# batra-mlp-lab/visdial

Hardware: NVIDIA H100
Metric: QA-rounds/sec mn-att-ques-im-hist+disc train step (higher is better)
Workload: dtype f16 operands + f16 saved state for the option LSTM, tf32 operands elsewhere; fp32 accumulate, fp32 cell state / gradients / optimiser

## Files before the change

visdial_b200/csrc/lstm16.cu:

```cuda
#include <cuda.h>
#include <cuda_fp16.h>
#include <map>
#include <mutex>
#include "../../include/visdial_b200.h"
#include "kernels.cuh"
#include "tc_ptx.cuh"

namespace vd {
namespace tc {

constexpr int BM16 = 128;
constexpr int BK16 = 64;
constexpr int UK16 = 16;
constexpr int BN16 = 128;
constexpr int EW16 = 8;
constexpr int STAGE16 = 32768;

__device__ __forceinline__ float tanh16(float x) { float y; asm("tanh.approx.f32 %0, %1;" : "=f"(y) : "f"(x)); return y; }
__device__ __forceinline__ float sig16(float x) { return fmaf(0.5f, tanh16(0.5f * x), 0.5f); }

__device__ __forceinline__ uint32_t pack2(float a, float b) {
  uint32_t r;
  asm("{\n .reg .f16 lo, hi;\n cvt.rn.satfinite.f16.f32 lo, %1;\n cvt.rn.satfinite.f16.f32 hi, %2;\n mov.b32 %0, {lo, hi};\n}"
      : "=r"(r) : "f"(a), "f"(b));
  return r;
}
__device__ __forceinline__ uint4 pack8(const float* v) {
  return make_uint4(pack2(v[0], v[1]), pack2(v[2], v[3]), pack2(v[4], v[5]), pack2(v[6], v[7]));
}
__device__ __forceinline__ void unpack8(const uint4 u, float* v) {
  const __half2* h = reinterpret_cast<const __half2*>(&u);
#pragma unroll
  for (int i = 0; i < 4; ++i) { const float2 f = __half22float2(h[i]); v[2 * i] = f.x; v[2 * i + 1] = f.y; }
}

constexpr int T16_BYTES = 1024, T32_BYTES = 2048;
__device__ __forceinline__ uint8_t* t16_at(uint8_t* base, int row, int unit) {
  return base + row * 64 + (((unit >> 3) ^ ((row >> 1) & 3)) << 4) + (unit & 7) * 2;
}
__device__ __forceinline__ uint8_t* t32_at(uint8_t* base, int row, int unit) {
  return base + row * 128 + (((unit >> 2) ^ (row & 7)) << 4) + (unit & 3) * 4;
}
__device__ __forceinline__ const void* shfl_vptr(const void* p, int src_lane) {
  unsigned long long v = (unsigned long long)p;
  unsigned lo = __shfl_sync(0xffffffffu, (unsigned)v, src_lane), hi = __shfl_sync(0xffffffffu, (unsigned)(v >> 32), src_lane);
  return (const void*)(((unsigned long long)hi << 32) | lo);
}
__device__ __forceinline__ void cp16(void* dst, const void* src) {
  asm volatile("cp.async.cg.shared.global [%0], [%1], 16;" ::"r"(smem_u32(dst)), "l"(src) : "memory");
}
__device__ __forceinline__ void t16_load(uint8_t* base, const void* mine, int lane) {
#pragma unroll
  for (int ps = 0; ps < 2; ++ps) {
    const int row = ps * 8 + (lane >> 2), c = lane & 3;
    const uint8_t* src = (const uint8_t*)shfl_vptr(mine, row);
    uint8_t* dst = base + row * 64 + ((c ^ ((row >> 1) & 3)) << 4);
    if (src) cp16(dst, src + c * 16); else *reinterpret_cast<uint4*>(dst) = make_uint4(0, 0, 0, 0);
  }
}
__device__ __forceinline__ void t32_load(uint8_t* base, const void* mine, int lane) {
#pragma unroll
  for (int ps = 0; ps < 4; ++ps) {
    const int row = ps * 4 + (lane >> 3), c = lane & 7;
    const uint8_t* src = (const uint8_t*)shfl_vptr(mine, row);
    uint8_t* dst = base + row * 128 + ((c ^ (row & 7)) << 4);
    if (src) cp16(dst, src + c * 16); else *reinterpret_cast<float4*>(dst) = make_float4(0.f, 0.f, 0.f, 0.f);
  }
}
__device__ __forceinline__ void cp_wait_all() {
  asm volatile("cp.async.wait_all;" ::: "memory");
  __syncwarp();
}
__device__ __forceinline__ float2 ld_h2(uint8_t* p) { return __half22float2(*reinterpret_cast<const __half2*>(p)); }
__device__ __forceinline__ void st_h2(uint8_t* p, float a, float b) { *reinterpret_cast<uint32_t*>(p) = pack2(a, b); }

struct Lstm16Params {
  int R, H;
  const __half* ptable; const int32_t* tok;
  const float* bias;
  const float* c_prev;
  const int32_t* mask_ids;
  float* h32_out;
  int save_gates;
  const __half* gsave; const float* c_cur; float* dc_carry;
};
struct Lstm16Maps { CUtensorMap g16, c, h16; };

template <int MODE>
struct Cfg16 {
  static constexpr int THREADS = 128 + 32 * EW16;
  static constexpr int STG_PER_WARP = MODE == 0 ? (5 * T16_BYTES + T32_BYTES) : (4 * T16_BYTES + 3 * T32_BYTES);
  static constexpr int STG_BYTES = EW16 * STG_PER_WARP;
  static constexpr int STAGES = (232448 - 1024 - 256 - STG_BYTES) / STAGE16;
  static constexpr int TOTAL = STAGES * STAGE16 + STG_BYTES + 1024 + 256;
};

template <int MODE>
__global__ void __launch_bounds__(Cfg16<MODE>::THREADS, 1)
k_lstm16(const __grid_constant__ CUtensorMap tmA, const __grid_constant__ CUtensorMap tmB,
         const __grid_constant__ Lstm16Maps em, const Lstm16Params p) {
  using C = Cfg16<MODE>;
  constexpr int STAGES = C::STAGES;
  extern __shared__ uint8_t smem_raw[];
  uint8_t* smem = (uint8_t*)(((uintptr_t)smem_raw + 1023) & ~(uintptr_t)1023);
  uint8_t* stg_all = smem + STAGES * STAGE16;
  uint64_t* full = (uint64_t*)(stg_all + C::STG_BYTES);
  uint64_t* empty = full + STAGES;

  const int warp = threadIdx.x >> 5, lane = threadIdx.x & 31;
  const int H = p.H;
  const int num_m = (p.R + BM16 - 1) / BM16;
  const int num_n = MODE == 0 ? H / 32 : H / BN16;
  const int num_tiles = num_m * num_n;
  const int num_kb = (MODE == 0 ? H : 4 * H) / BK16;

  if (threadIdx.x == 0) {
    for (int s = 0; s < STAGES; ++s) { mbar_init(&full[s], 1); mbar_init(&empty[s], 2); }
    asm volatile("fence.mbarrier_init.release.cluster;" ::: "memory");
  }
  __syncthreads();

  if (warp < 4) {
    if (threadIdx.x == 0) {
      int s = 0; uint32_t ph = 0;
      for (int tile = blockIdx.x; tile < num_tiles; tile += gridDim.x) {
        const int m0 = (tile / num_n) * BM16;
        const int nt = tile % num_n;
        for (int kb = 0; kb < num_kb; ++kb) {
          mbar_wait(&empty[s], ph ^ 1);
          uint8_t* sa = smem + s * STAGE16;
          uint8_t* sb = sa + 16384;
          mbar_expect_tx(&full[s], STAGE16);
          tma_load_2d(sa, &tmA, &full[s], kb * BK16, m0);
          if (MODE == 0) {
#pragma unroll
            for (int g = 0; g < 4; ++g) tma_load_2d(sb + g * 4096, &tmB, &full[s], kb * BK16, g * H + nt * 32);
          } else {
            tma_load_2d(sb, &tmB, &full[s], kb * BK16, nt * BN16);
          }
          if (++s == STAGES) { s = 0; ph ^= 1; }
        }
      }
    }
  } else {
    const int cw = warp - 4, wg = cw >> 2;
    uint8_t* stg = stg_all + cw * C::STG_PER_WARP;
    const int fr = lane >> 2, fu = 2 * (lane & 3);
    int s = 0; uint32_t ph = 0;
    auto contract = [&](float (&d)[BN16 / 2]) {
#pragma unroll
      for (int i = 0; i < BN16 / 2; ++i) d[i] = 0.f;
      int prev = -1;
      for (int kb = 0; kb < num_kb; ++kb) {
        mbar_wait(&full[s], ph);
        const uint32_t sa = smem_u32(smem + s * STAGE16);
        const uint64_t adesc = make_desc(sa + wg * 64 * 128, 16, 1024), bdesc = make_desc(sa + 16384, 16, 1024);
        wgmma_fence();
#pragma unroll
        for (int k = 0; k < BK16 / UK16; ++k)
          wgmma_f16_n128(d, adesc + (uint64_t)(k * 2), bdesc + (uint64_t)(k * 2), (kb | k) ? 1u : 0u);
        wgmma_commit();
        wgmma_wait<1>();
        if (prev >= 0 && (threadIdx.x & 127) == 0) mbar_arrive(&empty[prev]);
        prev = s;
        if (++s == STAGES) { s = 0; ph ^= 1; }
      }
      wgmma_wait<0>();
      wgmma_hold(d);
      if (prev >= 0 && (threadIdx.x & 127) == 0) mbar_arrive(&empty[prev]);
    };
    if constexpr (MODE == 0) {
      uint8_t* sG = stg; uint8_t* sH = stg + 4 * T16_BYTES; uint8_t* sC = sH + T16_BYTES;
      for (int tile = blockIdx.x; tile < num_tiles; tile += gridDim.x) {
        const int m0 = (tile / num_n) * BM16;
        const int nt = tile % num_n;
        const int r0 = m0 + wg * 64 + (cw & 3) * 16;
        const int j0 = nt * 32;
        const int64_t row = (int64_t)r0 + (lane & 15);
        const bool row_ok = row < p.R;
        const float keep = (row_ok && p.mask_ids && p.mask_ids[row] == 0) ? 0.f : 1.f;
        const int32_t tk = row_ok ? __ldg(p.tok + row) : 0;
        const __half* prow = tk != 0 ? p.ptable + (int64_t)tk * 4 * H + j0 : nullptr;
        const float* cprow = (row_ok && p.c_prev) ? p.c_prev + row * H + j0 : nullptr;
        if (lane == 0) bulk_wait_read0();
        __syncwarp();
#pragma unroll
        for (int g = 0; g < 4; ++g) t16_load(sG + g * T16_BYTES, prow ? prow + g * H : nullptr, lane);
        t32_load(sC, cprow, lane);
        float d[BN16 / 2];
        contract(d);
        cp_wait_all();
#pragma unroll
        for (int hh = 0; hh < 2; ++hh) {
          const int r = fr + 8 * hh;
          const float kp = __shfl_sync(0xffffffffu, keep, r);
          const int64_t grow = (int64_t)r0 + r;
#pragma unroll
          for (int jj = 0; jj < 4; ++jj) {
            const int u = 8 * jj + fu;
            float a[4][2], cp[2], hn[2];
#pragma unroll
            for (int g = 0; g < 4; ++g) {
              const float2 x = ld_h2(t16_at(sG + g * T16_BYTES, r, u));
              const float2 b = __ldg(reinterpret_cast<const float2*>(p.bias + g * H + j0 + u));
              a[g][0] = d[4 * (jj + 4 * g) + 2 * hh] + (x.x + b.x);
              a[g][1] = d[4 * (jj + 4 * g) + 2 * hh + 1] + (x.y + b.y);
            }
            const float2 c2 = *reinterpret_cast<const float2*>(t32_at(sC, r, u));
            cp[0] = c2.x; cp[1] = c2.y;
#pragma unroll
            for (int e = 0; e < 2; ++e) {
              const float gi = sig16(a[0][e]), gf = sig16(a[1][e]), go = sig16(a[2][e]), gg = tanh16(a[3][e]);
              const float c_ = (gf * cp[e] + gi * gg) * kp;
              a[0][e] = gi * kp; a[1][e] = gf * kp; a[2][e] = go * kp; a[3][e] = gg * kp;
              cp[e] = c_; hn[e] = go * tanh16(c_) * kp;
            }
#pragma unroll
            for (int g = 0; g < 4; ++g) st_h2(t16_at(sG + g * T16_BYTES, r, u), a[g][0], a[g][1]);
            *reinterpret_cast<float2*>(t32_at(sC, r, u)) = make_float2(cp[0], cp[1]);
            st_h2(t16_at(sH, r, u), hn[0], hn[1]);
            if (p.h32_out && grow < p.R)
              *reinterpret_cast<float2*>(p.h32_out + grow * H + j0 + u) = make_float2(hn[0], hn[1]);
          }
        }
        fence_proxy_async_smem();
        __syncwarp();
        if (lane == 0) {
          if (p.save_gates) {
#pragma unroll
            for (int g = 0; g < 4; ++g) tma_store_2d(&em.g16, sG + g * T16_BYTES, g * H + j0, r0);
          }
          tma_store_2d(&em.c, sC, j0, r0);
          tma_store_2d(&em.h16, sH, j0, r0);
          bulk_commit();
        }
        __syncwarp();
      }
    } else {
      uint8_t* sG = stg; uint8_t* sCP = stg + 4 * T16_BYTES; uint8_t* sCC = sCP + T32_BYTES; uint8_t* sDC = sCC + T32_BYTES;
      for (int tile = blockIdx.x; tile < num_tiles; tile += gridDim.x) {
        const int m0 = (tile / num_n) * BM16;
        const int nt = tile % num_n;
        const int r0 = m0 + wg * 64 + (cw & 3) * 16;
        const int64_t row = (int64_t)r0 + (lane & 15);
        const bool row_ok = row < p.R;
        const float keep = (row_ok && p.mask_ids && p.mask_ids[row] == 0) ? 0.f : 1.f;
        const __half* grow = row_ok ? p.gsave + row * 4 * H : nullptr;
        const float* cprow = (row_ok && p.c_prev) ? p.c_prev + row * H : nullptr;
        const float* ccrow = row_ok ? p.c_cur + row * H : nullptr;
        const float* dcrow = row_ok ? p.dc_carry + row * H : nullptr;
        auto fetch = [&](int j) {
          if (lane == 0) bulk_wait_read0();
          __syncwarp();
#pragma unroll
          for (int g = 0; g < 4; ++g) t16_load(sG + g * T16_BYTES, grow ? grow + g * H + j : nullptr, lane);
          t32_load(sCP, cprow ? cprow + j : nullptr, lane);
          t32_load(sCC, ccrow ? ccrow + j : nullptr, lane);
          t32_load(sDC, dcrow ? dcrow + j : nullptr, lane);
        };
        fetch(nt * BN16);
        float d[BN16 / 2];
        contract(d);
#pragma unroll
        for (int grp = 0; grp < BN16 / 32; ++grp) {
          const int j = nt * BN16 + grp * 32;
          if (grp > 0) fetch(j);
          cp_wait_all();
#pragma unroll
          for (int hh = 0; hh < 2; ++hh) {
            const int r = fr + 8 * hh;
            const float keep_r = __shfl_sync(0xffffffffu, keep, r);
#pragma unroll
            for (int jj = 0; jj < 4; ++jj) {
              const int u = 8 * jj + fu;
              float g[4][2], cp[2], cc[2], dc[2], out[4][2], dcn[2];
#pragma unroll
              for (int gg = 0; gg < 4; ++gg) {
                const float2 x = ld_h2(t16_at(sG + gg * T16_BYTES, r, u));
                g[gg][0] = x.x; g[gg][1] = x.y;
              }
              const float2 cp2 = *reinterpret_cast<const float2*>(t32_at(sCP, r, u));
              const float2 cc2 = *reinterpret_cast<const float2*>(t32_at(sCC, r, u));
              const float2 dc2 = *reinterpret_cast<const float2*>(t32_at(sDC, r, u));
              cp[0] = cp2.x; cp[1] = cp2.y; cc[0] = cc2.x; cc[1] = cc2.y; dc[0] = dc2.x; dc[1] = dc2.y;
#pragma unroll
              for (int e = 0; e < 2; ++e) {
                const float dh = d[4 * (4 * grp + jj) + 2 * hh + e];
                const float gi = g[0][e], gf = g[1][e], go = g[2][e], gg_ = g[3][e];
                const float tcv = tanh16(cc[e]);
                const float dd = (dc[e] + dh * go * (1.f - tcv * tcv)) * keep_r;
                const float dhe = dh * keep_r;
                out[0][e] = dd * gg_ * gi * (1.f - gi);
                out[1][e] = dd * cp[e] * gf * (1.f - gf);
                out[2][e] = dhe * tcv * go * (1.f - go);
                out[3][e] = dd * gi * (1.f - gg_ * gg_);
                dcn[e] = dd * gf;
              }
#pragma unroll
              for (int gg = 0; gg < 4; ++gg) st_h2(t16_at(sG + gg * T16_BYTES, r, u), out[gg][0], out[gg][1]);
              *reinterpret_cast<float2*>(t32_at(sDC, r, u)) = make_float2(dcn[0], dcn[1]);
            }
          }
          fence_proxy_async_smem();
          __syncwarp();
          if (lane == 0) {
#pragma unroll
            for (int gg = 0; gg < 4; ++gg) tma_store_2d(&em.g16, sG + gg * T16_BYTES, gg * H + j, r0);
            tma_store_2d(&em.c, sDC, j, r0);
            bulk_commit();
          }
          __syncwarp();
        }
      }
    }
    if (lane == 0) asm volatile("cp.async.bulk.wait_group 0;" ::: "memory");
  }
}

constexpr int A16_KB = 64;
constexpr int A16_BM = 128, A16_BN = 256;
constexpr int A16_THREADS = 384;
constexpr int A16_A_BYTES = (A16_BM / 64) * A16_KB * 128;
constexpr int A16_B_BYTES = (A16_BN / 64) * A16_KB * 128;
constexpr int A16_STAGE = A16_A_BYTES + A16_B_BYTES;
constexpr int A16_STAGES = 4;
constexpr int A16_TOTAL = A16_STAGES * A16_STAGE + 1024 + 256;
constexpr int A16_CHUNKS_PER_CTA = 24;
constexpr int A16_MIN_CHUNK = 32;
struct Atb16Params {
  int M, N, tiles_n, tiles, kbt;
  int chunk, num_chunks;
  float* C; int64_t ldc; const float* inv_scale;
  int* counter;
};

template <bool VEC4>
__global__ void __launch_bounds__(A16_THREADS, 1)
k_atb16(const __grid_constant__ CUtensorMap tmA, const __grid_constant__ CUtensorMap tmB, const Atb16Params p) {
  extern __shared__ uint8_t smem_raw[];
  uint8_t* smem = (uint8_t*)(((uintptr_t)smem_raw + 1023) & ~(uintptr_t)1023);
  uint64_t* full = (uint64_t*)(smem + A16_STAGES * A16_STAGE);
  uint64_t* empty = full + A16_STAGES;
  int* tag = (int*)(empty + A16_STAGES);
  const int warp = threadIdx.x >> 5;

  if (threadIdx.x == 0) {
    for (int s = 0; s < A16_STAGES; ++s) { mbar_init(&full[s], 1); mbar_init(&empty[s], 2); }
    asm volatile("fence.mbarrier_init.release.cluster;" ::: "memory");
  }
  __syncthreads();

  if (warp < 4) {
    if (threadIdx.x == 0) {
      int s = 0; uint32_t ph = 0;
      for (;;) {
        const int c = atomicAdd(p.counter, 1);
        if (c >= p.num_chunks) break;
        const int tile = c % p.tiles, kb0 = (c / p.tiles) * p.chunk, kb1 = min(p.kbt, kb0 + p.chunk);
        const int m0 = (tile / p.tiles_n) * A16_BM, n0 = (tile % p.tiles_n) * A16_BN;
        for (int kb = kb0; kb < kb1; ++kb) {
          const int krow = kb * A16_KB;
          mbar_wait(&empty[s], ph ^ 1);
          uint8_t* sa = smem + s * A16_STAGE;
          uint8_t* sb = sa + A16_A_BYTES;
          if (kb == kb0) tag[s] = c;
          mbar_expect_tx(&full[s], A16_STAGE);
#pragma unroll
          for (int b = 0; b < A16_BM / 64; ++b) tma_load_2d(sa + b * A16_KB * 128, &tmA, &full[s], m0 + b * 64, krow);
// ... 211 lines not shown
      float* o = out + (int64_t)tok * ncols + c0;
      red_add_v4(o, acc[0] * sc, acc[1] * sc, acc[2] * sc, acc[3] * sc);
      red_add_v4(o + 4, acc[4] * sc, acc[5] * sc, acc[6] * sc, acc[7] * sc);
    };
    for (int64_t p = p0; p < p1; ++p) {
      const int tok = sorted_tok[p];
      if (tok != cur) {
        flush(cur);
#pragma unroll
        for (int e = 0; e < 8; ++e) acc[e] = 0.f;
        cur = tok;
      }
      float v[8];
      unpack8(__ldcs(reinterpret_cast<const uint4*>(X + (int64_t)perm[p] * ldx + c0)), v);
#pragma unroll
      for (int e = 0; e < 8; ++e) acc[e] += v[e];
    }
    flush(cur);
  }
}

static CUtensorMap make_tmap16(const void* base, CUtensorMapDataType dt, int esize, int64_t rows, int64_t cols, int64_t ld,
                               int box_rows, int box_cols, CUtensorMapSwizzle swz) {
  CUtensorMap tm;
  cuuint64_t dims[2] = {(cuuint64_t)cols, (cuuint64_t)rows};
  cuuint64_t strides[1] = {(cuuint64_t)ld * esize};
  cuuint32_t box[2] = {(cuuint32_t)box_cols, (cuuint32_t)box_rows};
  cuuint32_t estr[2] = {1, 1};
  CUresult r = get_encode()(&tm, dt, 2, (void*)base, dims, strides, box, estr, CU_TENSOR_MAP_INTERLEAVE_NONE, swz,
                            CU_TENSOR_MAP_L2_PROMOTION_L2_256B, CU_TENSOR_MAP_FLOAT_OOB_FILL_NONE);
  if (r != CUDA_SUCCESS) {
    char buf[256];
    snprintf(buf, sizeof(buf), "cuTensorMapEncodeTiled (lstm16) failed (%d): base %p rows %lld cols %lld ld %lld box %dx%d", (int)r, base,
             (long long)rows, (long long)cols, (long long)ld, box_rows, box_cols);
    throw CudaError(-3, buf);
  }
  return tm;
}
static CUtensorMap tmap_h(const __half* base, int64_t rows, int64_t cols, int64_t ld, int box_rows, int box_cols,
                          CUtensorMapSwizzle swz) {
  return make_tmap16(base, CU_TENSOR_MAP_DATA_TYPE_FLOAT16, 2, rows, cols, ld, box_rows, box_cols, swz);
}
static CUtensorMap tmap_f(const float* base, int64_t rows, int64_t cols, int64_t ld, int box_rows, int box_cols,
                          CUtensorMapSwizzle swz) {
  return make_tmap16(base, CU_TENSOR_MAP_DATA_TYPE_FLOAT32, 4, rows, cols, ld, box_rows, box_cols, swz);
}

template <int MODE>
static void launch16(LaunchCtx& cx, const CUtensorMap& tA, const CUtensorMap& tB, const Lstm16Maps& em, const Lstm16Params& p,
                     int num_tiles) {
  using C = Cfg16<MODE>;
  static bool attr_set = false;
  if (!attr_set) {
    VD_CUDA_CHECK(cudaFuncSetAttribute(k_lstm16<MODE>, cudaFuncAttributeMaxDynamicSharedMemorySize, C::TOTAL));
    attr_set = true;
  }
  const int pmax = cx.sms();
  int grid = num_tiles;
  if (num_tiles > pmax) { const int rounds = cdiv(num_tiles, pmax); grid = cdiv(num_tiles, rounds); }
  k_lstm16<MODE><<<grid, C::THREADS, C::TOTAL, cx.stream>>>(tA, tB, em, p);
  check_launch(cx, "k_lstm16");
}

}

bool lstm16_shape_ok(int64_t R, int H) { return H % 256 == 0 && H <= 512 && R >= 1024; }

void lstm16_step_fwd(LaunchCtx& cx, int64_t R, int H, const __half* h_prev16, const __half* Wh16, const __half* ptable16,
                     const int32_t* tok, const float* bias, const float* c_prev, const int32_t* mask_ids, __half* gates16,
                     float* c_out, __half* h16_out, float* h32_out) {
  using namespace tc;
  VD_REQUIRE(lstm16_shape_ok(R, H), VD_E_STATE, "lstm16_step_fwd: shape");
  Lstm16Params p = {};
  p.R = (int)R; p.H = H; p.ptable = ptable16; p.tok = tok; p.bias = bias; p.c_prev = c_prev; p.mask_ids = mask_ids;
  p.h32_out = h32_out; p.save_gates = gates16 != nullptr;
  CUtensorMap tA = tmap_h(h_prev16, R, H, H, BM16, BK16, CU_TENSOR_MAP_SWIZZLE_128B);
  CUtensorMap tB = tmap_h(Wh16, 4 * (int64_t)H, H, H, 32, BK16, CU_TENSOR_MAP_SWIZZLE_128B);
  Lstm16Maps em;
  em.g16 = gates16 ? tmap_h(gates16, R, 4 * (int64_t)H, 4 * (int64_t)H, 16, 32, CU_TENSOR_MAP_SWIZZLE_64B)
                   : tmap_h(h16_out, R, H, H, 16, 32, CU_TENSOR_MAP_SWIZZLE_64B);
  em.c = tmap_f(c_out, R, H, H, 16, 32, CU_TENSOR_MAP_SWIZZLE_128B);
  em.h16 = tmap_h(h16_out, R, H, H, 16, 32, CU_TENSOR_MAP_SWIZZLE_64B);
  launch16<0>(cx, tA, tB, em, p, cdiv(R, BM16) * (H / 32));
}

void lstm16_step_bwd(LaunchCtx& cx, int64_t R, int H, const __half* da_next16, const __half* Whb16, const __half* gates16,
                     const float* c_prev, const float* c_cur, float* dc_carry, const int32_t* mask_ids, __half* da16) {
  using namespace tc;
  VD_REQUIRE(lstm16_shape_ok(R, H), VD_E_STATE, "lstm16_step_bwd: shape");
  Lstm16Params p = {};
  p.R = (int)R; p.H = H; p.gsave = gates16; p.c_prev = c_prev; p.c_cur = c_cur; p.dc_carry = dc_carry; p.mask_ids = mask_ids;
  CUtensorMap tA = tmap_h(da_next16, R, 4 * (int64_t)H, 4 * (int64_t)H, BM16, BK16, CU_TENSOR_MAP_SWIZZLE_128B);
  CUtensorMap tB = tmap_h(Whb16, H, 4 * (int64_t)H, 4 * (int64_t)H, 128, BK16, CU_TENSOR_MAP_SWIZZLE_128B);
  Lstm16Maps em;
  em.g16 = tmap_h(da16, R, 4 * (int64_t)H, 4 * (int64_t)H, 16, 32, CU_TENSOR_MAP_SWIZZLE_64B);
  em.c = tmap_f(dc_carry, R, H, H, 16, 32, CU_TENSOR_MAP_SWIZZLE_128B);
  em.h16 = em.c;
  launch16<1>(cx, tA, tB, em, p, cdiv(R, BM16) * (H / BN16));
}

void lstm16_first_step(LaunchCtx& cx, int64_t R, int H, const __half* ptable16, const int32_t* tok, const float* bias,
                       const float* c_prev, const int32_t* mask_ids, __half* gates16, float* c_out, __half* h16_out, float* h32_out) {
  const int64_t n = R * (H / 8);
  tc::k_lstm16_first<<<(unsigned)((n + 255) / 256), 256, 0, cx.stream>>>(ptable16, tok, bias, c_prev, mask_ids, gates16, c_out,
                                                                          h16_out, h32_out, R, H);
  check_launch(cx, "k_lstm16_first");
}

void lstm16_bwd_last(LaunchCtx& cx, int64_t R, int H, const __half* gates16, const float* c_prev, const float* c_cur,
                     const float* dh_last, const float* scale, const int32_t* mask_ids, float* dc_carry, __half* da16) {
  const int64_t n = R * (H / 8);
  tc::k_lstm16_bwd_last<<<(unsigned)((n + 255) / 256), 256, 0, cx.stream>>>(gates16, c_prev, c_cur, dh_last, scale, mask_ids,
                                                                             dc_carry, da16, R, H);
  check_launch(cx, "k_lstm16_bwd_last");
}

void cvt_f32_to_f16(LaunchCtx& cx, __half* dst, int64_t ldd, const float* src, int64_t lds, int64_t rows, int cols) {
  VD_REQUIRE(cols % 4 == 0 && lds % 4 == 0 && ldd % 4 == 0, VD_E_STATE, "cvt_f32_to_f16: alignment");
  const int64_t n = rows * (cols / 4);
  if (n == 0) return;
  tc::k_cvt16<<<(unsigned)((n + 255) / 256), 256, 0, cx.stream>>>(dst, ldd, src, lds, rows, cols);
  check_launch(cx, "k_cvt16");
}

void pick_grad_scale(LaunchCtx& cx, const float* x, int64_t n, uint32_t* bits, float* scale2) {
  VD_REQUIRE(n % 4 == 0, VD_E_STATE, "pick_grad_scale: n % 4");
  VD_CUDA_CHECK(cudaMemsetAsync(bits, 0, sizeof(uint32_t), cx.stream));
  const int blocks = (int)std::min<int64_t>((n / 4 + 255) / 256, 4 * cx.sm_count);
  tc::k_amax<<<blocks, 256, 0, cx.stream>>>(x, n / 4, bits);
  check_launch(cx, "k_amax");
  tc::k_pick_scale<<<1, 1, 0, cx.stream>>>(bits, scale2);
  check_launch(cx, "k_pick_scale");
}

void segsum_rows16(LaunchCtx& cx, const __half* X, int64_t ldx, const int32_t* perm, const int32_t* sorted_tok, int64_t n,
                   float* out, int ncols, const float* inv_scale) {
// ... 50 lines not shown
```

visdial_b200/csrc/tc_ptx.cuh:

```cuda
#pragma once
#include <cuda.h>
#include <stdint.h>

namespace vd {
namespace tc {

__device__ __forceinline__ uint32_t smem_u32(const void* p) { return (uint32_t)__cvta_generic_to_shared(p); }

__device__ __forceinline__ void mbar_init(uint64_t* bar, uint32_t count) {
  asm volatile("mbarrier.init.shared::cta.b64 [%0], %1;" ::"r"(smem_u32(bar)), "r"(count));
}
__device__ __forceinline__ void mbar_expect_tx(uint64_t* bar, uint32_t bytes) {
  asm volatile("mbarrier.arrive.expect_tx.shared::cta.b64 _, [%0], %1;" ::"r"(smem_u32(bar)), "r"(bytes) : "memory");
}
__device__ __forceinline__ void mbar_arrive(uint64_t* bar) {
  asm volatile("mbarrier.arrive.shared::cta.b64 _, [%0];" ::"r"(smem_u32(bar)) : "memory");
}
__device__ __forceinline__ void mbar_wait(uint64_t* bar, uint32_t parity) {
  uint32_t done = 0, spins = 0;
  uint32_t addr = smem_u32(bar);
  while (!done) {
    asm volatile(
        "{\n .reg .pred p;\n mbarrier.try_wait.parity.shared::cta.b64 p, [%1], %2;\n selp.u32 %0, 1, 0, p;\n}"
        : "=r"(done) : "r"(addr), "r"(parity) : "memory");
    if (!done && ++spins > (1u << 24)) __trap();
  }
}
__device__ __forceinline__ void tma_load_2d(void* smem_dst, const CUtensorMap* tm, uint64_t* bar, int c0, int c1) {
  asm volatile(
      "cp.async.bulk.tensor.2d.shared::cluster.global.mbarrier::complete_tx::bytes [%0], [%1, {%3, %4}], [%2];"
      ::"r"(smem_u32(smem_dst)), "l"(tm), "r"(smem_u32(bar)), "r"(c0), "r"(c1) : "memory");
}
__device__ __forceinline__ void wgmma_fence() { asm volatile("wgmma.fence.sync.aligned;" ::: "memory"); }
__device__ __forceinline__ void wgmma_commit() { asm volatile("wgmma.commit_group.sync.aligned;" ::: "memory"); }
template <int N> __device__ __forceinline__ void wgmma_wait() { asm volatile("wgmma.wait_group.sync.aligned %0;" ::"n"(N) : "memory"); }
template <int NR> __device__ __forceinline__ void wgmma_hold(float (&d)[NR]) {
#pragma unroll
  for (int i = 0; i < NR; ++i) asm volatile("" : "+f"(d[i])::"memory");
}
__device__ __forceinline__ void bar_named(int id, int threads) { asm volatile("bar.sync %0, %1;" ::"r"(id), "r"(threads) : "memory"); }

__device__ __forceinline__ uint64_t make_desc(uint32_t saddr, uint32_t lbo_bytes, uint32_t sbo_bytes) {
  uint64_t d = 0;
  d |= (uint64_t)((saddr & 0x3FFFF) >> 4);
  d |= (uint64_t)((lbo_bytes >> 4) & 0x3FFF) << 16;
  d |= (uint64_t)((sbo_bytes >> 4) & 0x3FFF) << 32;
  d |= (uint64_t)1 << 62;
  return d;
}

__device__ __forceinline__ void wgmma_tf32_n32(float (&d)[16], uint64_t a, uint64_t b, uint32_t acc) {
  asm volatile(
      "{\n .reg .pred p;\n setp.ne.b32 p, %18, 0;\n"
      "wgmma.mma_async.sync.aligned.m64n32k8.f32.tf32.tf32 {%0, %1, %2, %3, %4, %5, %6, %7, %8, %9, %10, %11, %12, %13, %14, %15}, %16, %17, p, 1, 1;\n}\n"
      : "+f"(d[0]), "+f"(d[1]), "+f"(d[2]), "+f"(d[3]), "+f"(d[4]), "+f"(d[5]), "+f"(d[6]), "+f"(d[7]), "+f"(d[8]), "+f"(d[9]), "+f"(d[10]), "+f"(d[11]), "+f"(d[12]), "+f"(d[13]), "+f"(d[14]), "+f"(d[15])
      : "l"(a), "l"(b), "r"(acc));
}

__device__ __forceinline__ void wgmma_tf32_n64(float (&d)[32], uint64_t a, uint64_t b, uint32_t acc) {
  asm volatile(
      "{\n .reg .pred p;\n setp.ne.b32 p, %34, 0;\n"
      "wgmma.mma_async.sync.aligned.m64n64k8.f32.tf32.tf32 {%0, %1, %2, %3, %4, %5, %6, %7, %8, %9, %10, %11, %12, %13, %14, %15, %16, %17, %18, %19, %20, %21, %22, %23, %24, %25, %26, %27, %28, %29, %30, %31}, %32, %33, p, 1, 1;\n}\n"
      : "+f"(d[0]), "+f"(d[1]), "+f"(d[2]), "+f"(d[3]), "+f"(d[4]), "+f"(d[5]), "+f"(d[6]), "+f"(d[7]), "+f"(d[8]), "+f"(d[9]), "+f"(d[10]), "+f"(d[11]), "+f"(d[12]), "+f"(d[13]), "+f"(d[14]), "+f"(d[15]), "+f"(d[16]), "+f"(d[17]), "+f"(d[18]), "+f"(d[19]), "+f"(d[20]), "+f"(d[21]), "+f"(d[22]), "+f"(d[23]), "+f"(d[24]), "+f"(d[25]), "+f"(d[26]), "+f"(d[27]), "+f"(d[28]), "+f"(d[29]), "+f"(d[30]), "+f"(d[31])
      : "l"(a), "l"(b), "r"(acc));
}

__device__ __forceinline__ void wgmma_tf32_n128(float (&d)[64], uint64_t a, uint64_t b, uint32_t acc) {
  asm volatile(
      "{\n .reg .pred p;\n setp.ne.b32 p, %66, 0;\n"
      "wgmma.mma_async.sync.aligned.m64n128k8.f32.tf32.tf32 {%0, %1, %2, %3, %4, %5, %6, %7, %8, %9, %10, %11, %12, %13, %14, %15, %16, %17, %18, %19, %20, %21, %22, %23, %24, %25, %26, %27, %28, %29, %30, %31, %32, %33, %34, %35, %36, %37, %38, %39, %40, %41, %42, %43, %44, %45, %46, %47, %48, %49, %50, %51, %52, %53, %54, %55, %56, %57, %58, %59, %60, %61, %62, %63}, %64, %65, p, 1, 1;\n}\n"
      : "+f"(d[0]), "+f"(d[1]), "+f"(d[2]), "+f"(d[3]), "+f"(d[4]), "+f"(d[5]), "+f"(d[6]), "+f"(d[7]), "+f"(d[8]), "+f"(d[9]), "+f"(d[10]), "+f"(d[11]), "+f"(d[12]), "+f"(d[13]), "+f"(d[14]), "+f"(d[15]), "+f"(d[16]), "+f"(d[17]), "+f"(d[18]), "+f"(d[19]), "+f"(d[20]), "+f"(d[21]), "+f"(d[22]), "+f"(d[23]), "+f"(d[24]), "+f"(d[25]), "+f"(d[26]), "+f"(d[27]), "+f"(d[28]), "+f"(d[29]), "+f"(d[30]), "+f"(d[31]), "+f"(d[32]), "+f"(d[33]), "+f"(d[34]), "+f"(d[35]), "+f"(d[36]), "+f"(d[37]), "+f"(d[38]), "+f"(d[39]), "+f"(d[40]), "+f"(d[41]), "+f"(d[42]), "+f"(d[43]), "+f"(d[44]), "+f"(d[45]), "+f"(d[46]), "+f"(d[47]), "+f"(d[48]), "+f"(d[49]), "+f"(d[50]), "+f"(d[51]), "+f"(d[52]), "+f"(d[53]), "+f"(d[54]), "+f"(d[55]), "+f"(d[56]), "+f"(d[57]), "+f"(d[58]), "+f"(d[59]), "+f"(d[60]), "+f"(d[61]), "+f"(d[62]), "+f"(d[63])
      : "l"(a), "l"(b), "r"(acc));
}

__device__ __forceinline__ void wgmma_f16_n32(float (&d)[16], uint64_t a, uint64_t b, uint32_t acc) {
  asm volatile(
      "{\n .reg .pred p;\n setp.ne.b32 p, %18, 0;\n"
      "wgmma.mma_async.sync.aligned.m64n32k16.f32.f16.f16 {%0, %1, %2, %3, %4, %5, %6, %7, %8, %9, %10, %11, %12, %13, %14, %15}, %16, %17, p, 1, 1, 0, 0;\n}\n"
      : "+f"(d[0]), "+f"(d[1]), "+f"(d[2]), "+f"(d[3]), "+f"(d[4]), "+f"(d[5]), "+f"(d[6]), "+f"(d[7]), "+f"(d[8]), "+f"(d[9]), "+f"(d[10]), "+f"(d[11]), "+f"(d[12]), "+f"(d[13]), "+f"(d[14]), "+f"(d[15])
      : "l"(a), "l"(b), "r"(acc));
}

__device__ __forceinline__ void wgmma_f16_n128(float (&d)[64], uint64_t a, uint64_t b, uint32_t acc) {
  asm volatile(
      "{\n .reg .pred p;\n setp.ne.b32 p, %66, 0;\n"
      "wgmma.mma_async.sync.aligned.m64n128k16.f32.f16.f16 {%0, %1, %2, %3, %4, %5, %6, %7, %8, %9, %10, %11, %12, %13, %14, %15, %16, %17, %18, %19, %20, %21, %22, %23, %24, %25, %26, %27, %28, %29, %30, %31, %32, %33, %34, %35, %36, %37, %38, %39, %40, %41, %42, %43, %44, %45, %46, %47, %48, %49, %50, %51, %52, %53, %54, %55, %56, %57, %58, %59, %60, %61, %62, %63}, %64, %65, p, 1, 1, 0, 0;\n}\n"
      : "+f"(d[0]), "+f"(d[1]), "+f"(d[2]), "+f"(d[3]), "+f"(d[4]), "+f"(d[5]), "+f"(d[6]), "+f"(d[7]), "+f"(d[8]), "+f"(d[9]), "+f"(d[10]), "+f"(d[11]), "+f"(d[12]), "+f"(d[13]), "+f"(d[14]), "+f"(d[15]), "+f"(d[16]), "+f"(d[17]), "+f"(d[18]), "+f"(d[19]), "+f"(d[20]), "+f"(d[21]), "+f"(d[22]), "+f"(d[23]), "+f"(d[24]), "+f"(d[25]), "+f"(d[26]), "+f"(d[27]), "+f"(d[28]), "+f"(d[29]), "+f"(d[30]), "+f"(d[31]), "+f"(d[32]), "+f"(d[33]), "+f"(d[34]), "+f"(d[35]), "+f"(d[36]), "+f"(d[37]), "+f"(d[38]), "+f"(d[39]), "+f"(d[40]), "+f"(d[41]), "+f"(d[42]), "+f"(d[43]), "+f"(d[44]), "+f"(d[45]), "+f"(d[46]), "+f"(d[47]), "+f"(d[48]), "+f"(d[49]), "+f"(d[50]), "+f"(d[51]), "+f"(d[52]), "+f"(d[53]), "+f"(d[54]), "+f"(d[55]), "+f"(d[56]), "+f"(d[57]), "+f"(d[58]), "+f"(d[59]), "+f"(d[60]), "+f"(d[61]), "+f"(d[62]), "+f"(d[63])
      : "l"(a), "l"(b), "r"(acc));
}

__device__ __forceinline__ void wgmma_f16_n256_mn(float (&d)[128], uint64_t a, uint64_t b, uint32_t acc) {
  asm volatile(
      "{\n .reg .pred p;\n setp.ne.b32 p, %130, 0;\n"
// ... 51 lines not shown
```

Measured before the change: 16240.

## Keep weight tile resident and ping-pong warpgroups in forward LSTM16 step

In the training forward step (when gates are saved), the B (recurrent weight) slice for a tile is loaded once into dedicated shared-memory slots and reused by both 64-row halves. The two consumer warpgroups take turns on the MMA via turn barriers, so one group's epilogue can overlap the other's contraction. A-stages shrink to 64-row tiles, which allows more pipeline stages. The inference path moves to a new MODE 2 that keeps the old behaviour. This adds barrier complexity and serialises the MMA between warpgroups, which could cost throughput if the epilogue is short.

```diff
diff --git a/visdial_b200/csrc/lstm16.cu b/visdial_b200/csrc/lstm16.cu
--- a/visdial_b200/csrc/lstm16.cu
+++ b/visdial_b200/csrc/lstm16.cu
@@ -89,10 +89,12 @@
 template <int MODE>
 struct Cfg16 {
   static constexpr int THREADS = 128 + 32 * EW16;
-  static constexpr int STG_PER_WARP = MODE == 0 ? (5 * T16_BYTES + T32_BYTES) : (4 * T16_BYTES + 3 * T32_BYTES);
+  static constexpr int STG_PER_WARP = MODE != 1 ? (5 * T16_BYTES + T32_BYTES) : (4 * T16_BYTES + 3 * T32_BYTES);
   static constexpr int STG_BYTES = EW16 * STG_PER_WARP;
-  static constexpr int STAGES = (232448 - 1024 - 256 - STG_BYTES) / STAGE16;
-  static constexpr int TOTAL = STAGES * STAGE16 + STG_BYTES + 1024 + 256;
+  static constexpr int STAGE = MODE == 0 ? 8192 : STAGE16;
+  static constexpr int B_SLOTS = MODE == 0 ? 8 : 0, B_SLOT = 16384;
+  static constexpr int STAGES = (232448 - 1024 - 256 - STG_BYTES - B_SLOTS * B_SLOT) / STAGE;
+  static constexpr int TOTAL = STAGES * STAGE + B_SLOTS * B_SLOT + STG_BYTES + 1024 + 256;
 };
 
 template <int MODE>
@@ -103,25 +105,56 @@
   constexpr int STAGES = C::STAGES;
   extern __shared__ uint8_t smem_raw[];
   uint8_t* smem = (uint8_t*)(((uintptr_t)smem_raw + 1023) & ~(uintptr_t)1023);
-  uint8_t* stg_all = smem + STAGES * STAGE16;
+  uint8_t* bslot = smem + STAGES * C::STAGE;
+  uint8_t* stg_all = bslot + C::B_SLOTS * C::B_SLOT;
   uint64_t* full = (uint64_t*)(stg_all + C::STG_BYTES);
   uint64_t* empty = full + STAGES;
+  uint64_t* bfull = empty + STAGES;
+  uint64_t* bempty = bfull + C::B_SLOTS;
+  uint64_t* turn = bempty + C::B_SLOTS;
 
   const int warp = threadIdx.x >> 5, lane = threadIdx.x & 31;
   const int H = p.H;
   const int num_m = (p.R + BM16 - 1) / BM16;
-  const int num_n = MODE == 0 ? H / 32 : H / BN16;
+  const int num_n = MODE != 1 ? H / 32 : H / BN16;
   const int num_tiles = num_m * num_n;
-  const int num_kb = (MODE == 0 ? H : 4 * H) / BK16;
+  const int num_kb = (MODE != 1 ? H : 4 * H) / BK16;
 
   if (threadIdx.x == 0) {
-    for (int s = 0; s < STAGES; ++s) { mbar_init(&full[s], 1); mbar_init(&empty[s], 2); }
+    for (int s = 0; s < STAGES; ++s) { mbar_init(&full[s], 1); mbar_init(&empty[s], MODE == 0 ? 1 : 2); }
+    for (int s = 0; s < C::B_SLOTS; ++s) { mbar_init(&bfull[s], 1); mbar_init(&bempty[s], 2); }
+    if (MODE == 0) { mbar_init(&turn[0], 4); mbar_init(&turn[1], 4); }
     asm volatile("fence.mbarrier_init.release.cluster;" ::: "memory");
   }
   __syncthreads();
 
   if (warp < 4) {
-    if (threadIdx.x == 0) {
+    if (threadIdx.x == 0 && MODE == 0) {
+      int s = 0; uint32_t ph = 0, bph = 0;
+      for (int tile = blockIdx.x; tile < num_tiles; tile += gridDim.x, bph ^= 1) {
+        const int m0 = (tile / num_n) * BM16;
+        const int nt = tile % num_n;
+        for (int half = 0; half < 2; ++half) {
+          for (int kb = 0; kb < num_kb; ++kb) {
+            if (half == 0) {
+              mbar_wait(&bempty[kb], bph ^ 1);
+              uint8_t* sb = bslot + kb * C::B_SLOT;
+              mbar_expect_tx(&bfull[kb], C::B_SLOT);
+#pragma unroll
+              for (int g = 0; g < 4; ++g) tma_load_2d(sb + g * 4096, &tmB, &bfull[kb], kb * BK16, g * H + nt * 32);
+            }
+            mbar_wait(&empty[s], ph ^ 1);
+            if (m0 + half * 64 < p.R) {
+              mbar_expect_tx(&full[s], C::STAGE);
+              tma_load_2d(smem + s * C::STAGE, &tmA, &full[s], kb * BK16, m0 + half * 64);
+            } else {
+              mbar_arrive(&full[s]);
+            }
+            if (++s == STAGES) { s = 0; ph ^= 1; }
+          }
+        }
+      }
+    } else if (threadIdx.x == 0) {
       int s = 0; uint32_t ph = 0;
       for (int tile = blockIdx.x; tile < num_tiles; tile += gridDim.x) {
         const int m0 = (tile / num_n) * BM16;
@@ -129,14 +162,13 @@
         for (int kb = 0; kb < num_kb; ++kb) {
           mbar_wait(&empty[s], ph ^ 1);
           uint8_t* sa = smem + s * STAGE16;
-          uint8_t* sb = sa + 16384;
           mbar_expect_tx(&full[s], STAGE16);
           tma_load_2d(sa, &tmA, &full[s], kb * BK16, m0);
-          if (MODE == 0) {
-#pragma unroll
-            for (int g = 0; g < 4; ++g) tma_load_2d(sb + g * 4096, &tmB, &full[s], kb * BK16, g * H + nt * 32);
+          if (MODE == 2) {
+#pragma unroll
+            for (int g = 0; g < 4; ++g) tma_load_2d(sa + 16384 + g * 4096, &tmB, &full[s], kb * BK16, g * H + nt * 32);
           } else {
-            tma_load_2d(sb, &tmB, &full[s], kb * BK16, nt * BN16);
+            tma_load_2d(sa + 16384, &tmB, &full[s], kb * BK16, nt * BN16);
           }
           if (++s == STAGES) { s = 0; ph ^= 1; }
         }
@@ -169,9 +201,12 @@
       wgmma_hold(d);
       if (prev >= 0 && (threadIdx.x & 127) == 0) mbar_arrive(&empty[prev]);
     };
-    if constexpr (MODE == 0) {
+    if constexpr (MODE != 1) {
       uint8_t* sG = stg; uint8_t* sH = stg + 4 * T16_BYTES; uint8_t* sC = sH + T16_BYTES;
-      for (int tile = blockIdx.x; tile < num_tiles; tile += gridDim.x) {
+      auto skip = [&]() { s += num_kb; while (s >= STAGES) { s -= STAGES; ph ^= 1; } };
+      if (MODE == 0 && wg == 1) skip();
+      uint32_t tp = 0;
+      for (int tile = blockIdx.x; tile < num_tiles; tile += gridDim.x, tp ^= 1) {
         const int m0 = (tile / num_n) * BM16;
         const int nt = tile % num_n;
         const int r0 = m0 + wg * 64 + (cw & 3) * 16;
@@ -188,7 +223,35 @@
         for (int g = 0; g < 4; ++g) t16_load(sG + g * T16_BYTES, prow ? prow + g * H : nullptr, lane);
         t32_load(sC, cprow, lane);
         float d[BN16 / 2];
-        contract(d);
+        if constexpr (MODE == 0) {
+#pragma unroll
+          for (int i = 0; i < BN16 / 2; ++i) d[i] = 0.f;
+          mbar_wait(&turn[wg], tp ^ (wg == 0 ? 1u : 0u));
+          int prev = -1;
+          for (int kb = 0; kb < num_kb; ++kb) {
+            mbar_wait(&bfull[kb], tp);
+            mbar_wait(&full[s], ph);
+            const uint64_t adesc = make_desc(smem_u32(smem + s * C::STAGE), 16, 1024);
+            const uint64_t bdesc = make_desc(smem_u32(bslot + kb * C::B_SLOT), 16, 1024);
+            wgmma_fence();
+#pragma unroll
+            for (int k = 0; k < BK16 / UK16; ++k)
+              wgmma_f16_n128(d, adesc + (uint64_t)(k * 2), bdesc + (uint64_t)(k * 2), (kb | k) ? 1u : 0u);
+            wgmma_commit();
+            wgmma_wait<1>();
+            if (prev >= 0 && (threadIdx.x & 127) == 0) { mbar_arrive(&empty[prev]); mbar_arrive(&bempty[kb - 1]); }
+            prev = s;
+            if (++s == STAGES) { s = 0; ph ^= 1; }
+          }
+          __syncwarp();
+          if (lane == 0) mbar_arrive(&turn[wg ^ 1]);
+          wgmma_wait<0>();
+          wgmma_hold(d);
+          if ((threadIdx.x & 127) == 0) { mbar_arrive(&empty[prev]); mbar_arrive(&bempty[num_kb - 1]); }
+          skip();
+        } else {
+          contract(d);
+        }
         cp_wait_all();
 #pragma unroll
         for (int hh = 0; hh < 2; ++hh) {
@@ -653,14 +716,15 @@
   Lstm16Params p = {};
   p.R = (int)R; p.H = H; p.ptable = ptable16; p.tok = tok; p.bias = bias; p.c_prev = c_prev; p.mask_ids = mask_ids;
   p.h32_out = h32_out; p.save_gates = gates16 != nullptr;
-  CUtensorMap tA = tmap_h(h_prev16, R, H, H, BM16, BK16, CU_TENSOR_MAP_SWIZZLE_128B);
+  CUtensorMap tA = tmap_h(h_prev16, R, H, H, gates16 ? 64 : BM16, BK16, CU_TENSOR_MAP_SWIZZLE_128B);
   CUtensorMap tB = tmap_h(Wh16, 4 * (int64_t)H, H, H, 32, BK16, CU_TENSOR_MAP_SWIZZLE_128B);
   Lstm16Maps em;
   em.g16 = gates16 ? tmap_h(gates16, R, 4 * (int64_t)H, 4 * (int64_t)H, 16, 32, CU_TENSOR_MAP_SWIZZLE_64B)
                    : tmap_h(h16_out, R, H, H, 16, 32, CU_TENSOR_MAP_SWIZZLE_64B);
   em.c = tmap_f(c_out, R, H, H, 16, 32, CU_TENSOR_MAP_SWIZZLE_128B);
   em.h16 = tmap_h(h16_out, R, H, H, 16, 32, CU_TENSOR_MAP_SWIZZLE_64B);
-  launch16<0>(cx, tA, tB, em, p, cdiv(R, BM16) * (H / 32));
+  if (gates16) launch16<0>(cx, tA, tB, em, p, cdiv(R, BM16) * (H / 32));
+  else launch16<2>(cx, tA, tB, em, p, cdiv(R, BM16) * (H / 32));
 }
 
 void lstm16_step_bwd(LaunchCtx& cx, int64_t R, int H, const __half* da_next16, const __half* Whb16, const __half* gates16,
```

After: 16350, median of 6. Within noise of the previous version (+0.7%).

## Overlap LSTM16 forward epilogue with next tile's WGMMA using double accumulators

Applied to the files above, without the earlier changes.

The forward option-LSTM kernel now keeps two accumulator sets and interleaves the next tile's wgmma issues into the gate/cell epilogue of the current tile, and prefetches the next tile's side inputs early. The producer warpgroup gives up registers via setmaxnreg so the consumers can hold both accumulators. The hidden size also becomes a template parameter so the K loop count is known at compile time, and barrier waits set a flag instead of trapping inline. This hides epilogue latency behind tensor-core work, at the cost of register pressure and more complex stage release bookkeeping.

```diff
diff --git a/visdial_b200/csrc/lstm16.cu b/visdial_b200/csrc/lstm16.cu
--- a/visdial_b200/csrc/lstm16.cu
+++ b/visdial_b200/csrc/lstm16.cu
@@ -73,6 +73,17 @@
 }
 __device__ __forceinline__ float2 ld_h2(uint8_t* p) { return __half22float2(*reinterpret_cast<const __half2*>(p)); }
 __device__ __forceinline__ void st_h2(uint8_t* p, float a, float b) { *reinterpret_cast<uint32_t*>(p) = pack2(a, b); }
+
+__device__ __forceinline__ void mbar_wait_flag(uint64_t* bar, uint32_t parity, uint32_t& stuck) {
+  uint32_t done = 0, spins = 0;
+  const uint32_t addr = smem_u32(bar);
+  while (!done) {
+    asm volatile(
+        "{\n .reg .pred p;\n mbarrier.try_wait.parity.shared::cta.b64 p, [%1], %2;\n selp.u32 %0, 1, 0, p;\n}"
+        : "=r"(done) : "r"(addr), "r"(parity) : "memory");
+    if (!done && ++spins > (1u << 24)) { stuck = 1; break; }
+  }
+}
 
 struct Lstm16Params {
   int R, H;
@@ -95,7 +106,7 @@
   static constexpr int TOTAL = STAGES * STAGE16 + STG_BYTES + 1024 + 256;
 };
 
-template <int MODE>
+template <int MODE, int HID>
 __global__ void __launch_bounds__(Cfg16<MODE>::THREADS, 1)
 k_lstm16(const __grid_constant__ CUtensorMap tmA, const __grid_constant__ CUtensorMap tmB,
          const __grid_constant__ Lstm16Maps em, const Lstm16Params p) {
@@ -108,11 +119,11 @@
   uint64_t* empty = full + STAGES;
 
   const int warp = threadIdx.x >> 5, lane = threadIdx.x & 31;
-  const int H = p.H;
+  constexpr int H = HID;
   const int num_m = (p.R + BM16 - 1) / BM16;
   const int num_n = MODE == 0 ? H / 32 : H / BN16;
   const int num_tiles = num_m * num_n;
-  const int num_kb = (MODE == 0 ? H : 4 * H) / BK16;
+  constexpr int num_kb = (MODE == 0 ? H : 4 * H) / BK16;
 
   if (threadIdx.x == 0) {
     for (int s = 0; s < STAGES; ++s) { mbar_init(&full[s], 1); mbar_init(&empty[s], 2); }
@@ -120,7 +131,9 @@
   }
   __syncthreads();
 
-  if (warp < 4) {
+  const int wgroup = __shfl_sync(0xffffffffu, threadIdx.x / 128, 0);
+  if (wgroup == 0) {
+    setmaxnreg_dec<40>();
     if (threadIdx.x == 0) {
       int s = 0; uint32_t ph = 0;
       for (int tile = blockIdx.x; tile < num_tiles; tile += gridDim.x) {
@@ -143,52 +156,78 @@
       }
     }
   } else {
+    setmaxnreg_inc<232>();
     const int cw = warp - 4, wg = cw >> 2;
     uint8_t* stg = stg_all + cw * C::STG_PER_WARP;
     const int fr = lane >> 2, fu = 2 * (lane & 3);
-    int s = 0; uint32_t ph = 0;
-    auto contract = [&](float (&d)[BN16 / 2]) {
+    const bool lead = (threadIdx.x & 127) == 0;
+    int s = 0, rs = 0, held = 0; uint32_t ph = 0;
+    uint32_t stuck = 0;
+    auto issue = [&](float (&d)[BN16 / 2], int kb) {
+      mbar_wait_flag(&full[s], ph, stuck);
+      const uint32_t sa = smem_u32(smem + s * STAGE16);
+      const uint64_t adesc = make_desc(sa + wg * 64 * 128, 16, 1024), bdesc = make_desc(sa + 16384, 16, 1024);
+      wgmma_fence();
+#pragma unroll
+      for (int k = 0; k < BK16 / UK16; ++k)
+        wgmma_f16_n128(d, adesc + (uint64_t)(k * 2), bdesc + (uint64_t)(k * 2), (kb | k) ? 1u : 0u);
+      wgmma_commit();
+      if (++s == STAGES) { s = 0; ph ^= 1; }
+      ++held;
+    };
+    auto release = [&](int keep) {
+      for (; held > keep; --held) {
+        if (lead) mbar_arrive(&empty[rs]);
+        if (++rs == STAGES) rs = 0;
+      }
+    };
+    auto zero = [](float (&d)[BN16 / 2]) {
 #pragma unroll
       for (int i = 0; i < BN16 / 2; ++i) d[i] = 0.f;
-      int prev = -1;
-      for (int kb = 0; kb < num_kb; ++kb) {
-        mbar_wait(&full[s], ph);
-        const uint32_t sa = smem_u32(smem + s * STAGE16);
-        const uint64_t adesc = make_desc(sa + wg * 64 * 128, 16, 1024), bdesc = make_desc(sa + 16384, 16, 1024);
-        wgmma_fence();
-#pragma unroll
-        for (int k = 0; k < BK16 / UK16; ++k)
-          wgmma_f16_n128(d, adesc + (uint64_t)(k * 2), bdesc + (uint64_t)(k * 2), (kb | k) ? 1u : 0u);
-        wgmma_commit();
-        wgmma_wait<1>();
-        if (prev >= 0 && (threadIdx.x & 127) == 0) mbar_arrive(&empty[prev]);
-        prev = s;
-        if (++s == STAGES) { s = 0; ph ^= 1; }
-      }
-      wgmma_wait<0>();
-      wgmma_hold(d);
-      if (prev >= 0 && (threadIdx.x & 127) == 0) mbar_arrive(&empty[prev]);
     };
-    if constexpr (MODE == 0) {
-      uint8_t* sG = stg; uint8_t* sH = stg + 4 * T16_BYTES; uint8_t* sC = sH + T16_BYTES;
-      for (int tile = blockIdx.x; tile < num_tiles; tile += gridDim.x) {
-        const int m0 = (tile / num_n) * BM16;
-        const int nt = tile % num_n;
-        const int r0 = m0 + wg * 64 + (cw & 3) * 16;
+    float keep = 1.f;
+    auto bwd_fetch = [&](int tile, int j) {
+      const int64_t row = (int64_t)(tile / num_n) * BM16 + wg * 64 + (cw & 3) * 16 + (lane & 15);
+      const bool row_ok = row < p.R;
+      const __half* grow = row_ok ? p.gsave + row * 4 * H : nullptr;
+      const float* cprow = (row_ok && p.c_prev) ? p.c_prev + row * H : nullptr;
+      const float* ccrow = row_ok ? p.c_cur + row * H : nullptr;
+      const float* dcrow = row_ok ? p.dc_carry + row * H : nullptr;
+      uint8_t* sG = stg; uint8_t* sCP = stg + 4 * T16_BYTES; uint8_t* sCC = sCP + T32_BYTES; uint8_t* sDC = sCC + T32_BYTES;
+      if (lane == 0) bulk_wait_read0();
+      __syncwarp();
+#pragma unroll
+      for (int g = 0; g < 4; ++g) t16_load(sG + g * T16_BYTES, grow ? grow + g * H + j : nullptr, lane);
+      t32_load(sCP, cprow ? cprow + j : nullptr, lane);
+      t32_load(sCC, ccrow ? ccrow + j : nullptr, lane);
+      t32_load(sDC, dcrow ? dcrow + j : nullptr, lane);
+    };
+    auto fetch = [&](int tile) {
+      const int m0 = (tile / num_n) * BM16, nt = tile % num_n;
+      const int64_t row = (int64_t)m0 + wg * 64 + (cw & 3) * 16 + (lane & 15);
+      const bool row_ok = row < p.R;
+      keep = (row_ok && p.mask_ids && p.mask_ids[row] == 0) ? 0.f : 1.f;
+      if constexpr (MODE == 0) {
         const int j0 = nt * 32;
-        const int64_t row = (int64_t)r0 + (lane & 15);
-        const bool row_ok = row < p.R;
-        const float keep = (row_ok && p.mask_ids && p.mask_ids[row] == 0) ? 0.f : 1.f;
         const int32_t tk = row_ok ? __ldg(p.tok + row) : 0;
         const __half* prow = tk != 0 ? p.ptable + (int64_t)tk * 4 * H + j0 : nullptr;
         const float* cprow = (row_ok && p.c_prev) ? p.c_prev + row * H + j0 : nullptr;
         if (lane == 0) bulk_wait_read0();
         __syncwarp();
+        uint8_t* sG = stg; uint8_t* sC = stg + 5 * T16_BYTES;
 #pragma unroll
         for (int g = 0; g < 4; ++g) t16_load(sG + g * T16_BYTES, prow ? prow + g * H : nullptr, lane);
         t32_load(sC, cprow, lane);
-        float d[BN16 / 2];
-        contract(d);
+      } else {
+        bwd_fetch(tile, nt * BN16);
+      }
+    };
+    auto epilogue = [&](float (&d)[BN16 / 2], int tile, auto&& tick) {
+      const int m0 = (tile / num_n) * BM16, nt = tile % num_n;
+      const int r0 = m0 + wg * 64 + (cw & 3) * 16;
+      if constexpr (MODE == 0) {
+        uint8_t* sG = stg; uint8_t* sH = stg + 4 * T16_BYTES; uint8_t* sC = sH + T16_BYTES;
+        const int j0 = nt * 32;
         cp_wait_all();
 #pragma unroll
         for (int hh = 0; hh < 2; ++hh) {
@@ -221,6 +260,7 @@
             st_h2(t16_at(sH, r, u), hn[0], hn[1]);
             if (p.h32_out && grow < p.R)
               *reinterpret_cast<float2*>(p.h32_out + grow * H + j0 + u) = make_float2(hn[0], hn[1]);
+            tick(4 * hh + jj);
           }
         }
         fence_proxy_async_smem();
@@ -235,36 +275,12 @@
           bulk_commit();
         }
         __syncwarp();
-      }
-    } else {
-      uint8_t* sG = stg; uint8_t* sCP = stg + 4 * T16_BYTES; uint8_t* sCC = sCP + T32_BYTES; uint8_t* sDC = sCC + T32_BYTES;
-      for (int tile = blockIdx.x; tile < num_tiles; tile += gridDim.x) {
-        const int m0 = (tile / num_n) * BM16;
-        const int nt = tile % num_n;
-        const int r0 = m0 + wg * 64 + (cw & 3) * 16;
-        const int64_t row = (int64_t)r0 + (lane & 15);
-        const bool row_ok = row < p.R;
-        const float keep = (row_ok && p.mask_ids && p.mask_ids[row] == 0) ? 0.f : 1.f;
-        const __half* grow = row_ok ? p.gsave + row * 4 * H : nullptr;
-        const float* cprow = (row_ok && p.c_prev) ? p.c_prev + row * H : nullptr;
-        const float* ccrow = row_ok ? p.c_cur + row * H : nullptr;
-        const float* dcrow = row_ok ? p.dc_carry + row * H : nullptr;
-        auto fetch = [&](int j) {
-          if (lane == 0) bulk_wait_read0();
-          __syncwarp();
-#pragma unroll
-          for (int g = 0; g < 4; ++g) t16_load(sG + g * T16_BYTES, grow ? grow + g * H + j : nullptr, lane);
-          t32_load(sCP, cprow ? cprow + j : nullptr, lane);
-          t32_load(sCC, ccrow ? ccrow + j : nullptr, lane);
-          t32_load(sDC, dcrow ? dcrow + j : nullptr, lane);
-        };
-        fetch(nt * BN16);
-        float d[BN16 / 2];
-        contract(d);
+      } else {
+        uint8_t* sG = stg; uint8_t* sCP = stg + 4 * T16_BYTES; uint8_t* sCC = sCP + T32_BYTES; uint8_t* sDC = sCC + T32_BYTES;
 #pragma unroll
         for (int grp = 0; grp < BN16 / 32; ++grp) {
           const int j = nt * BN16 + grp * 32;
-          if (grp > 0) fetch(j);
+          if (grp > 0) bwd_fetch(tile, j);
           cp_wait_all();
 #pragma unroll
           for (int hh = 0; hh < 2; ++hh) {
@@ -299,6 +315,7 @@
 #pragma unroll
               for (int gg = 0; gg < 4; ++gg) st_h2(t16_at(sG + gg * T16_BYTES, r, u), out[gg][0], out[gg][1]);
               *reinterpret_cast<float2*>(t32_at(sDC, r, u)) = make_float2(dcn[0], dcn[1]);
+              tick(8 * grp + 4 * hh + jj);
             }
           }
           fence_proxy_async_smem();
@@ -312,8 +329,69 @@
           __syncwarp();
         }
       }
+    };
+    constexpr int TAIL16 = 2;
+    constexpr int LIM = num_kb - TAIL16;
+    auto step = [&](float (&x)[BN16 / 2], float (&y)[BN16 / 2], int tile) {
+      const int next = tile + gridDim.x;
+      issue(y, 0);
+      wgmma_wait<1>();
+      wgmma_hold(x);
+      release(1);
+      epilogue(x, tile, [&](int piece) {
+        if (piece + 1 < LIM) {
+          issue(y, piece + 1);
+          wgmma_wait<1>();
+          release(1);
+        }
+      });
+      fetch(next);
+#pragma unroll
+      for (int kb = LIM > 1 ? LIM : 1; kb < num_kb; ++kb) {
+        issue(y, kb);
+        wgmma_wait<1>();
+        release(1);
+      }
+      return next;
+    };
+    auto last = [&](float (&x)[BN16 / 2], int tile) {
+      wgmma_wait<0>();
+      wgmma_hold(x);
+      release(0);
+      epilogue(x, tile, [](int) {});
+    };
+    int tile = blockIdx.x;
+    if constexpr (MODE == 1) {
+      for (; tile < num_tiles; tile += gridDim.x) {
+        float d[BN16 / 2];
+        fetch(tile);
+        zero(d);
+        for (int kb = 0; kb < num_kb; ++kb) {
+          issue(d, kb);
+          wgmma_wait<1>();
+          release(1);
+        }
+        last(d, tile);
+      }
+    } else if (tile < num_tiles) {
+      float d0[BN16 / 2], d1[BN16 / 2];
+      fetch(tile);
+      zero(d0);
+      zero(d1);
+      for (int kb = 0; kb < num_kb; ++kb) {
+        issue(d0, kb);
+        wgmma_wait<1>();
+        release(1);
+      }
+      for (;;) {
+        if (tile + (int)gridDim.x >= num_tiles) { last(d0, tile); break; }
+        tile = step(d0, d1, tile);
+        if (tile + (int)gridDim.x >= num_tiles) { last(d1, tile); break; }
+        tile = step(d1, d0, tile);
+      }
     }
     if (lane == 0) asm volatile("cp.async.bulk.wait_group 0;" ::: "memory");
+    if (stuck) __trap();
   }
 }
 
@@ -631,13 +709,16 @@
   using C = Cfg16<MODE>;
   static bool attr_set = false;
   if (!attr_set) {
-    VD_CUDA_CHECK(cudaFuncSetAttribute(k_lstm16<MODE>, cudaFuncAttributeMaxDynamicSharedMemorySize, C::TOTAL));
+    VD_CUDA_CHECK(cudaFuncSetAttribute(k_lstm16<MODE, 256>, cudaFuncAttributeMaxDynamicSharedMemorySize, C::TOTAL));
+    VD_CUDA_CHECK(cudaFuncSetAttribute(k_lstm16<MODE, 512>, cudaFuncAttributeMaxDynamicSharedMemorySize, C::TOTAL));
     attr_set = true;
   }
   const int pmax = cx.sms();
   int grid = num_tiles;
   if (num_tiles > pmax) { const int rounds = cdiv(num_tiles, pmax); grid = cdiv(num_tiles, rounds); }
-  k_lstm16<MODE><<<grid, C::THREADS, C::TOTAL, cx.stream>>>(tA, tB, em, p);
+  VD_REQUIRE(p.H == 256 || p.H == 512, VD_E_STATE, "k_lstm16: H");
+  if (p.H == 256) k_lstm16<MODE, 256><<<grid, C::THREADS, C::TOTAL, cx.stream>>>(tA, tB, em, p);
+  else k_lstm16<MODE, 512><<<grid, C::THREADS, C::TOTAL, cx.stream>>>(tA, tB, em, p);
   check_launch(cx, "k_lstm16");
 }
 
diff --git a/visdial_b200/csrc/tc_ptx.cuh b/visdial_b200/csrc/tc_ptx.cuh
--- a/visdial_b200/csrc/tc_ptx.cuh
+++ b/visdial_b200/csrc/tc_ptx.cuh
@@ -39,6 +39,8 @@
   for (int i = 0; i < NR; ++i) asm volatile("" : "+f"(d[i])::"memory");
 }
 __device__ __forceinline__ void bar_named(int id, int threads) { asm volatile("bar.sync %0, %1;" ::"r"(id), "r"(threads) : "memory"); }
+template <int N> __device__ __forceinline__ void setmaxnreg_dec() { asm volatile("setmaxnreg.dec.sync.aligned.u32 %0;" ::"n"(N)); }
+template <int N> __device__ __forceinline__ void setmaxnreg_inc() { asm volatile("setmaxnreg.inc.sync.aligned.u32 %0;" ::"n"(N)); }
 
 __device__ __forceinline__ uint64_t make_desc(uint32_t saddr, uint32_t lbo_bytes, uint32_t sbo_bytes) {
   uint64_t d = 0;
```

Result: faster. 16210 before, 16500 after, median of 6 (+1.8%).
